# rojas-diego/tokengeex

Measured on NVIDIA B200. Metric: encode_input_throughput, higher is better.
Workload: dtype f64 scores / u32 ids

## Files before the change

### tokengeex_b200/csrc/tgx_api.cu

```cuda
#include <cub/cub.cuh>
#include <cuda_runtime.h>

#include <algorithm>
#include <cmath>
#include <cstdio>
#include <cstdlib>
#include <cstring>
#include <ctime>
#include <memory>
#include <mutex>
#include <string>
#include <thread>
#include <vector>

#include "../../include/tokengeex_b200.h"
#include "tgx_kernels.cuh"
#include "tgx_match_kernels.cuh"
#include "tgx_team_kernel.cuh"
#include "tgx_fb_rows_kernels.cuh"
#include "trie_build.h"

namespace {

thread_local std::string g_err;
// ... 704 lines not shown
  if (m->device < 0) return TGX_OK;
  cudaStream_t st = m->w().stream;
  tgx::TokenHash h;
  bool hash_ok = V != 0 && max_token_len >= 1 && max_token_len <= 16;
  if (hash_ok && built) {
    hash_ok = built_err->empty();
    if (hash_ok) h = std::move(*built);
  } else if (hash_ok) {
    hash_ok = tgx::build_token_hash(token_bytes, token_offsets, V, &h).empty();
  }
  if (hash_ok) CU(m->d_hash.reserve(h.slots.size() * sizeof(tgx::Slot)));
  m->hash.mask = 0;
  m->hash.slots.clear();
  m->have_rows = false;
  if (hash_ok) {
    CU(cudaMemcpyAsync(m->d_hash.p, h.slots.data(), h.slots.size() * sizeof(tgx::Slot), cudaMemcpyHostToDevice, st));
    CU(cudaStreamSynchronize(st));
    m->hash = std::move(h);
  }
  return TGX_OK;
}

int ensure_match_tables(tgx_model* m) {
  if (m->have_rows || m->device < 0) return TGX_OK;
  if (!tgx::build_match_tables(&m->da).empty()) return TGX_OK;
  const tgx::DoubleArray& da = m->da;
  cudaStream_t st = m->w().stream;
  CU(m->d_trie8.reserve(da.slots8.size() * 8));
  CU(m->d_rows.reserve(da.rows.size() * 8 + 256));
  CU(m->d_rowids.reserve(da.row_ids.size() * 4 + 256));
  CU(cudaMemcpyAsync(m->d_trie8.p, da.slots8.data(), da.slots8.size() * 8, cudaMemcpyHostToDevice, st));
  CU(cudaMemcpyAsync(m->d_rows.p, da.rows.data(), da.rows.size() * 8, cudaMemcpyHostToDevice, st));
  CU(cudaMemcpyAsync(m->d_rowids.p, da.row_ids.data(), da.row_ids.size() * 4, cudaMemcpyHostToDevice, st));
  CU(m->d_pair2.reserve(da.pair2.size() * 8));
  CU(cudaMemcpyAsync(m->d_pair2.p, da.pair2.data(), da.pair2.size() * 8, cudaMemcpyHostToDevice, st));
  CU(cudaStreamSynchronize(st));
  m->have_rows = true;
  m->rows16 = (uint32_t)(da.rows.size() / 2);
  return TGX_OK;
}

int run_crlf(tgx_model* m, const uint8_t* d_text, const uint64_t* d_off, uint64_t S, uint64_t N) {
  cudaStream_t st = m->w().stream;
  uint64_t n_tiles = (N + CRLF_TILE - 1) / CRLF_TILE;
  CU(m->w().text2.reserve(N + 16));
  CU(m->w().off2.reserve((S + 1) * 8));
  CU(m->w().bitmap.reserve((N / 32 + 4) * 4));
  CU(m->w().blk.reserve((n_tiles + 1) * 8 * 2));
  CU(dev_fill(m->w().bitmap.p, 0, (N / 32 + 4) * 4, st));
  if (S > 1) {
    crlf_mark_starts<<<nblk(S, 256), 256, 0, st>>>(d_off, S, m->w().bitmap.as<uint32_t>());
    m->w().stats.launches += 1;
  }
  unsigned long long* removed = m->w().blk.as<unsigned long long>();
  unsigned long long* prefix = removed + n_tiles + 1;
  CU(dev_fill(removed, 0, (n_tiles + 1) * 8, st));
  if (n_tiles) {
    crlf_count<<<(uint32_t)n_tiles, CRLF_BLOCK, 0, st>>>(d_text, N, m->w().bitmap.as<uint32_t>(), removed);
    m->w().stats.launches += 1;
  }
  size_t tmp = 0;
  CU(cub::DeviceScan::ExclusiveSum(nullptr, tmp, removed, prefix, (int)(n_tiles + 1), st));
  CU(m->w().cubtmp.reserve(tmp));
  CU(cub::DeviceScan::ExclusiveSum(m->w().cubtmp.p, tmp, removed, prefix, (int)(n_tiles + 1), st));
  m->w().stats.launches += 2;
  if (n_tiles) {
    crlf_scatter<<<(uint32_t)n_tiles, CRLF_BLOCK, 0, st>>>(d_text, N, d_off, S, m->w().bitmap.as<uint32_t>(), prefix,
                                                          n_tiles, m->w().text2.as<uint8_t>(), m->w().off2.as<uint64_t>());
    m->w().stats.launches += 1;
  } else {
    CU(dev_fill(m->w().off2.p, 0, (S + 1) * 8, st));
  }
  CU(cudaGetLastError());
  return TGX_OK;
}

int sort_units(tgx_model* m, uint32_t U) {
  CU(m->w().keys_out.reserve((size_t)U * 4 + 4));
  CU(m->w().vals_out.reserve((size_t)U * 4 + 4));
  size_t tmp = 0;
  CU(cub::DeviceRadixSort::SortPairsDescending(nullptr, tmp, m->w().ulen.as<uint32_t>(), m->w().keys_out.as<uint32_t>(),
                                               m->w().vals_in.as<uint32_t>(), m->w().vals_out.as<uint32_t>(), (int)U, 0, 32,
                                               m->w().stream));
  CU(m->w().cubtmp.reserve(tmp));
  CU(cub::DeviceRadixSort::SortPairsDescending(m->w().cubtmp.p, tmp, m->w().ulen.as<uint32_t>(), m->w().keys_out.as<uint32_t>(),
                                               m->w().vals_in.as<uint32_t>(), m->w().vals_out.as<uint32_t>(), (int)U, 0, 32,
                                               m->w().stream));
  m->w().stats.launches += 4;
  return TGX_OK;
}

int read_words(tgx_model* m, const void* d0, const void* d1, unsigned long long* o0, unsigned long long* o1);

int run_match(tgx_model* m, const uint8_t* d_text, uint64_t N, const uint8_t* d_skip = nullptr) {
  cudaStream_t st = m->w().stream;
  CU(m->w().rec.reserve((N + 64) * 4));
  MatchParams mp;
  mp.text = d_text;
  mp.blob_end = d_text + N;
  mp.N = N;
  mp.trie8 = m->d_trie8.as<uint2>();
  mp.root_base = m->da.root_base;
  mp.rec = m->w().rec.as<uint32_t>();
  mp.skip = d_skip;
  mp.pair2 = m->d_pair2.as<uint2>();
  mp.slice = 0;
  const size_t budget = (size_t)std::min<int64_t>(m->match_stage_bytes, (int64_t)m->smem_optin - 1024);
  mp.staged = (uint32_t)std::min<size_t>(m->da.slots8.size(), budget / 8);
  const size_t smem = (size_t)mp.staged * 8;
  auto launch = [&](auto kernel, int ilp) -> cudaError_t {
    const uint32_t threads = (uint32_t)std::min(m->match_threads, mk_max_threads(ilp));
    cudaError_t e = cudaFuncSetAttribute(kernel, cudaFuncAttributeMaxDynamicSharedMemorySize, (int)smem);
    if (e != cudaSuccess) return e;
    const uint64_t per_cta = (uint64_t)threads * ilp;
    const uint64_t want = (uint64_t)m->num_sms * (uint64_t)std::max(1, m->match_ctas_per_sm);
    const uint64_t rounds = std::max<uint64_t>(1, (N + per_cta * want - 1) / (per_cta * want));
    mp.slice = rounds * per_cta;
    const uint32_t grid = (uint32_t)((N + mp.slice - 1) / mp.slice);
    kernel<<<grid, threads, smem, st>>>(mp);
    return cudaGetLastError();
  };
  if (m->match_compact) {
    const uint32_t threads = MK2_THREADS;
    const size_t qbytes = (size_t)(threads / 32) * 2 * MK2_Q * 8;
    const size_t budget2 = (size_t)std::min<int64_t>(m->match_stage_bytes, (int64_t)m->smem_optin - 1024 - (int64_t)qbytes);
    mp.staged = (uint32_t)std::min<size_t>(m->da.slots8.size(), budget2 / 8);
    const size_t smem2 = (size_t)mp.staged * 8 + qbytes;
    CU(cudaFuncSetAttribute(match2_kernel, cudaFuncAttributeMaxDynamicSharedMemorySize, (int)smem2));
    const uint64_t per_cta = (uint64_t)threads * 4;
    const uint64_t want = (uint64_t)m->num_sms * (uint64_t)std::max(1, m->match_ctas_per_sm);
    const uint64_t rounds = std::max<uint64_t>(1, (N + per_cta * want - 1) / (per_cta * want));
    mp.slice = rounds * per_cta;
    match2_kernel<<<(uint32_t)((N + mp.slice - 1) / mp.slice), threads, smem2, st>>>(mp);
    CU(cudaGetLastError());
    m->w().stats.launches += 1;
    return TGX_OK;
  }
  CU(launch(match_kernel<4>, 4));
  m->w().stats.launches += 1;
  return TGX_OK;
}

int run_viterbi(tgx_model* m, const uint8_t* d_text, const uint64_t* d_off, uint64_t S, uint64_t N,
                uint64_t* d_proc_len, bool with_dropout = false) {
  cudaStream_t st = m->w().stream;
  if (S >= (1ull << 32)) return fail(TGX_ERR_INVALID, "too many samples in one call (< 2^32)");
  uint32_t U = (uint32_t)S;
  const uint64_t n_tiles = (N + EM_TILE - 1) / EM_TILE;
  CU(m->w().ustart.reserve((size_t)U * 8 + 8));
  CU(m->w().ulen.reserve((size_t)U * 4 + 4));
  CU(m->w().vals_in.reserve((size_t)U * 4 + 4));
  CU(m->w().bp.reserve(N + 64));
  CU(m->w().mark.reserve(n_tiles * EM_TILE + 64));
  CU(m->w().ntok.reserve(((size_t)U + 1) * 8));
  CU(m->w().status.reserve((size_t)U * 4 + 4));
  CU(m->w().small.reserve(256));
  units_from_samples<<<nblk(U, 256), 256, 0, st>>>(d_off, S, m->w().ustart.as<uint64_t>(), m->w().ulen.as<uint32_t>(),
                                                  m->w().vals_in.as<uint32_t>(), d_proc_len);
  m->w().stats.launches += 1;
  int rc = sort_units(m, U);
  if (rc) return rc;
  uint32_t* counts = m->w().small.as<uint32_t>();
  uint32_t thr = (uint32_t)std::min<int64_t>(m->long_threshold, 0x7FFFFFFF);
  const uint32_t thr2 = (uint32_t)std::min<int64_t>(m->team_long_threshold, 0x7FFFFFFF);
  split_sorted<<<1, 32, 0, st>>>(m->w().keys_out.as<uint32_t>(), U, thr, thr2, counts);
  m->w().stats.launches += 1;
  CU(dev_fill(m->w().ntok.p, 0, ((size_t)U + 1) * 8, st));
  CU(dev_fill(m->w().status.p, 0, (size_t)U * 4 + 4, st));
  CU(dev_fill(m->w().mark.p, 0, n_tiles * EM_TILE, st));

  UnitParams u;
  u.text = d_text;
  u.unit_start = m->w().ustart.as<uint64_t>();
  u.unit_len = m->w().ulen.as<uint32_t>();
  u.order = m->w().vals_out.as<uint32_t>();
  u.trie = m->d_trie;
  u.root_base = m->da.root_base;
  u.rows = std::max<uint32_t>(1, m->da.max_token_len);
  u.W = u.rows + 1;
  u.counts = counts;
  u.first = 0;
  u.count = U;

  const double dropout = with_dropout ? m->dropout : 0.0;
  const int algo_req = m->algo == 4 ? (with_dropout && N >= m->wide_bytes && u.rows <= 16 ? 3 : 2) : m->algo;
  if (!(dropout > 0.0) && (algo_req == 0 || algo_req == 3) && u.rows <= 16) {
    rc = ensure_match_tables(m);
    if (rc) return rc;
  }
  const int algo = dropout > 0.0 ? (algo_req == 1 ? 1 : 2) : ((algo_req == 0 || algo_req == 3) && !m->have_rows ? 2 : algo_req);
  m->w().algo_used = algo;
  m->w().side_used = false;
  uint32_t n_long = 0;
  if (algo == 3 && u.rows <= 16 && N && U) {
    unsigned long long w01 = 0, w23 = 0;
    rc = read_words(m, counts, counts + 2, &w01, &w23);
    if (rc) return rc;
    n_long = std::min<uint32_t>((uint32_t)w23, (uint32_t)(w01 >> 32));
  }
  CU(cudaEventRecord(m->w().ev[8], st));
  if ((algo == 0 || algo == 3) && u.rows <= 16 && N) {
    const uint8_t* d_skip = nullptr;
    if (algo == 3 && n_long && m->match_compact && m->match_skip) {
      const size_t nb = (size_t)((N + 127) >> 7);
      CU(m->w().skip.reserve(nb + 64));
      CU(dev_fill(m->w().skip.p, 0, nb, st));
      mark_skip_kernel<<<nblk((uint64_t)n_long * 32, 256), 256, 0, st>>>(u.unit_start, u.unit_len, u.order, n_long,
                                                                        m->w().skip.as<uint8_t>());
      m->w().stats.launches += 1;
      d_skip = m->w().skip.as<uint8_t>();
    }
    rc = run_match(m, d_text, N, d_skip);
    if (rc) return rc;
  }
  CU(cudaEventRecord(m->w().ev[9], st));
  CU(cudaEventRecord(m->w().ev[0], st));
  if (algo == 3 && u.rows <= 16) {
    if (N && U) {
      const uint32_t per_cta = (uint32_t)std::max(1, m->side_load);
      const uint32_t P = n_long ? std::min<uint32_t>((n_long + per_cta - 1) / per_cta, (uint32_t)m->num_sms * 2u / 3u) : 0u;
      unsigned int* ctr = m->w().small.as<unsigned int>() + 8;
      CU(dev_fill(ctr, 0, 8, st));
      CU(cudaEventRecord(m->w().ev_side_fork, st));
      if (P) {
        CU(cudaStreamWaitEvent(m->w().stream_side, m->w().ev_side_fork, 0));
        PairParams pp;
        pp.u = u;
        pp.u.part = 3;
        pp.u.count = n_long;
        pp.blob_end = d_text + N;
        pp.bp = m->w().bp.as<uint8_t>();
        pp.counter = ctr;
        pp.dbg = 0;
        m->w().side_used = true;
        CU(cudaEventRecord(m->w().ev[10], m->w().stream_side));
        {
          cudaStream_t keep = m->w().stream;
          m->w().stream = m->w().stream_side;
          m->pair_grid_cap = P;
          const int keep_groups = m->groups;
          if (m->side_groups > 0) m->groups = m->groups > 0 ? std::min(m->groups, m->side_groups) : m->side_groups;
          cudaError_t e = launch_viterbi_pair_r<2>(m, pp, 0);
          m->groups = keep_groups;
          m->pair_grid_cap = 0;
          m->w().stream = keep;
          CU(e);
        }
        CU(cudaEventRecord(m->w().ev[11], m->w().stream_side));
        CU(cudaEventRecord(m->w().ev_side_join, m->w().stream_side));
        CU(cudaStreamWaitEvent(m->w().stream_low, m->w().ev_side_fork, 0));
      }
      TeamParams tm;
      tm.u = u;
      tm.u.part = 4;
      tm.u.count = U - std::min(U, n_long);
      tm.rec = m->w().rec.as<uint32_t>();
      tm.rows = m->d_rows.as<double>();
      tm.bp = m->w().bp.as<uint8_t>();
      tm.counter = m->w().small.as<unsigned int>() + 9;
      const size_t budget = (size_t)std::min<int64_t>(m->team_hot_bytes, (int64_t)m->smem_optin - 1024);
      tm.hot16 = (uint32_t)std::max<size_t>(std::min<size_t>(m->rows16, budget / 16), std::min<size_t>(m->rows16, 9));
      const size_t smem = (size_t)tm.hot16 * 16;
      const uint32_t n_short = tm.u.count;
      if (n_short) {
        constexpr uint32_t warps = TM_WARPS, per_warp = 8;
        CU(cudaFuncSetAttribute(viterbi_team_kernel<warps>, cudaFuncAttributeMaxDynamicSharedMemorySize, (int)smem));
        const uint32_t ctas = ((n_short + per_warp - 1) / per_warp + warps - 1) / warps;
        const uint32_t g1 = std::max<uint32_t>(1, std::min<uint32_t>(ctas, (uint32_t)m->num_sms - P));
        viterbi_team_kernel<warps><<<g1, warps * 32, smem, st>>>(tm);
        m->w().stats.launches += 1;
        if (P && ctas > g1) {
          viterbi_team_kernel<warps><<<std::min<uint32_t>(ctas - g1, P), warps * 32, smem, m->w().stream_low>>>(tm);
          m->w().stats.launches += 1;
        }
        CU(cudaGetLastError());
      }
      if (P) {
        CU(cudaEventRecord(m->w().ev_low_join, m->w().stream_low));
        CU(cudaStreamWaitEvent(st, m->w().ev_low_join, 0));
      }
    }
  } else if (algo == 0 && u.rows <= 16) {
    if (N && U) {
      RowsParams rp;
      rp.u = u;
      rp.u.part = 0;
      rp.rec = m->w().rec.as<uint32_t>();
      rp.rows = m->d_rows.as<double>();
      const size_t budget = (size_t)std::min<int64_t>(m->rows_hot_bytes, (int64_t)m->smem_optin - 1024);
      rp.hot16 = (uint32_t)std::min<size_t>(m->rows16, budget / 16);
      rp.bp = m->w().bp.as<uint8_t>();
      rp.counter = m->w().small.as<unsigned int>() + 8;
      const size_t smem = (size_t)rp.hot16 * 16;
      CU(cudaFuncSetAttribute(viterbi_rows_kernel, cudaFuncAttributeMaxDynamicSharedMemorySize, (int)smem));
      CU(dev_fill(rp.counter, 0, 4, st));
      const uint32_t warps = (uint32_t)std::max(1, std::min(16, m->rows_warps));
      const uint32_t grid = (uint32_t)std::min<uint64_t>(((uint64_t)U + 2 * warps - 1) / (2 * warps), (uint64_t)m->num_sms);
      viterbi_rows_kernel<<<grid, warps * 32, smem, st>>>(rp);
      m->w().stats.launches += 1;
      CU(cudaGetLastError());
    }
  } else if (algo == 2 && u.rows <= 16) {
    PairParams p;
    p.u = u;
    p.u.part = 0;
    p.blob_end = d_text + N;
    p.bp = m->w().bp.as<uint8_t>();
    p.counter = m->w().small.as<unsigned int>() + 8;
    p.dbg = 0;
    DropInfo di;
    di.dropout = dropout;
    di.seed = m->drop_seed;
    di.unit_base = m->drop_unit_base;
    if (!p.u.count) {
    } else {
      CU(launch_viterbi_pair_r<2>(m, p, N, di));
    }
  } else {
    ViterbiParams p;
    p.u = u;
    p.bp = m->w().bp.as<uint8_t>();
    p.dropout = dropout;
    p.drop_seed = m->drop_seed;
    p.unit_base = m->drop_unit_base;
    p.u.part = 1;
    CU(launch_viterbi_g(m, 32, p));
    p.u.part = 2;
    CU(launch_viterbi_g(m, m->g_short, p));
  }
  CU(cudaEventRecord(m->w().ev[1], st));
  if (m->w().side_used) CU(cudaStreamWaitEvent(st, m->w().ev_side_join, 0));
  CU(cudaEventRecord(m->w().ev[12], st));
  CU(cudaEventRecord(m->w().ev[2], st));
  if (U) {
    BacktrackParams b;
    b.unit_start = u.unit_start;
    b.unit_len = u.unit_len;
    b.order = u.order;
    b.counts = counts;
    b.first = 0;
    b.count = U;
    b.bp = m->w().bp.as<uint8_t>();
    b.mark = m->w().mark.as<uint8_t>();
    b.n_tokens = m->w().ntok.as<unsigned long long>();
    b.status = m->w().status.as<int32_t>();
    b.part = 1;
    backtrack_warp_kernel<<<nblk(U, BW_WARPS), BW_WARPS * 32, 0, st>>>(b);
    b.part = 2;
    backtrack_thread_kernel<<<nblk(U, BT_THREADS), BT_THREADS, 0, st>>>(b);
    m->w().stats.launches += 2;
    CU(cudaGetLastError());
  }
  CU(cudaEventRecord(m->w().ev[3], st));
  return TGX_OK;
}

int run_emit(tgx_model* m, const uint8_t* d_text, uint64_t N, uint32_t* d_ids, uint64_t ids_cap,
             unsigned long long* d_freq) {
  cudaStream_t st = m->w().stream;
  const uint64_t n_tiles = (N + EM_TILE - 1) / EM_TILE;
  CU(cudaEventRecord(m->w().ev[4], st));
  if (n_tiles) {
    CU(m->w().tilecnt.reserve((n_tiles + 1) * 16));
    unsigned long long* cnt = m->w().tilecnt.as<unsigned long long>();
    unsigned long long* prefix = cnt + n_tiles + 1;
    const uint32_t grid = (uint32_t)std::min<uint64_t>(n_tiles, (uint64_t)m->num_sms * 8);
    mark_count_kernel<<<grid, EM_BLOCK, 0, st>>>(m->w().mark.as<uint4>(), n_tiles, cnt);
    size_t tmp = 0;
    CU(cub::DeviceScan::ExclusiveSum(nullptr, tmp, cnt, prefix, (int)n_tiles, st));
    CU(m->w().cubtmp.reserve(tmp));
    CU(cub::DeviceScan::ExclusiveSum(m->w().cubtmp.p, tmp, cnt, prefix, (int)n_tiles, st));
    EmitParams e;
    e.mark = m->w().mark.as<uint4>();
    e.text = d_text;
    e.text_bytes = N;
    e.n_tiles = n_tiles;
    e.tile_prefix = prefix;
    e.trie = m->d_trie;
    e.root_base = m->da.root_base;
    e.ids = d_ids;
    e.cap = ids_cap;
    e.freq = d_freq;
    e.V = (uint32_t)m->V;
    const bool use_hash = m->emit_hash && m->hash.mask != 0;
    e.hash = use_hash ? m->d_hash.as<uint4>() : nullptr;
    e.hash_mask = use_hash ? m->hash.mask : 0;
    e.hash_seed = m->hash.seed;
    emit_kernel<<<grid, EM_BLOCK, d_freq ? EM_HOT * 4 : 0, st>>>(e);
    m->w().stats.launches += 4;
    CU(cudaGetLastError());
  }
  CU(cudaEventRecord(m->w().ev[5], st));
  return TGX_OK;
}

int read_words(tgx_model* m, const void* d0, const void* d1, unsigned long long* o0, unsigned long long* o1) {
  CU(cudaEventRecord(m->w().ev_ctl, m->w().stream));
  CU(cudaStreamWaitEvent(m->w().stream_ctl, m->w().ev_ctl, 0));
  if (d0) CU(cudaMemcpyAsync(m->w().h_words, d0, 8, cudaMemcpyDeviceToHost, m->w().stream_ctl));
  if (d1) CU(cudaMemcpyAsync(m->w().h_words + 1, d1, 8, cudaMemcpyDeviceToHost, m->w().stream_ctl));
  CU(cudaStreamSynchronize(m->w().stream_ctl));
  if (d0 && o0) *o0 = m->w().h_words[0];
  if (d1 && o1) *o1 = m->w().h_words[1];
  return TGX_OK;
}

int first_bad(tgx_model* m, uint32_t U, int64_t* out_idx, const void* extra = nullptr, unsigned long long* extra_out = nullptr) {
  unsigned long long* d = m->w().small.as<unsigned long long>() + 2;
  CU(dev_fill(d, 0xFF, 8, m->w().stream));
  if (U) {
    first_bad_unit<<<nblk(U, 256), 256, 0, m->w().stream>>>(m->w().status.as<int32_t>(), U, d);
    m->w().stats.launches += 1;
  }
  unsigned long long h = ~0ull;
  int rc = read_words(m, d, extra, &h, extra_out);
  if (rc) return rc;
  *out_idx = (h == ~0ull) ? -1 : (int64_t)h;
  return TGX_OK;
}

void finish_stats(tgx_model* m, int which) {
  float ms = 0;
  if (cudaEventElapsedTime(&ms, m->w().ev[0], m->w().ev[1]) == cudaSuccess) {
    if (which == 1) m->w().stats.viterbi_ms = ms;
    if (which == 2) m->w().stats.fwd_ms = ms;
  }
  if (which == 2 && cudaEventElapsedTime(&ms, m->w().ev[2], m->w().ev[3]) == cudaSuccess) m->w().stats.bwd_ms = ms;
  if (which == 1 && cudaEventElapsedTime(&ms, m->w().ev[2], m->w().ev[3]) == cudaSuccess) m->w().stats.back_ms = ms;
  if (which == 1 && cudaEventElapsedTime(&ms, m->w().ev[4], m->w().ev[5]) == cudaSuccess) m->w().stats.emit_ms = ms;
  if (which == 1 && cudaEventElapsedTime(&ms, m->w().ev[8], m->w().ev[9]) == cudaSuccess) m->w().stats.match_ms = ms;
  if (which == 1 && cudaEventElapsedTime(&ms, m->w().ev[8], m->w().ev[12]) == cudaSuccess) m->w().stats.forward_ms = ms;
  if (which == 1) m->w().stats.algo = m->w().algo_used;
  if (which == 1 && m->w().side_used && cudaEventElapsedTime(&ms, m->w().ev[10], m->w().ev[11]) == cudaSuccess) m->w().stats.side_ms = ms;
  if (cudaEventElapsedTime(&ms, m->w().ev[6], m->w().ev[7]) == cudaSuccess) m->w().stats.total_ms = ms;
  m->last_stats = m->w().stats;
}

}

extern "C" {

const char* tgx_last_error(void) { return g_err.c_str(); }

int tgx_model_create(const uint8_t* token_bytes, const uint64_t* token_offsets, const double* scores,
                     uint64_t vocab_size, int device, tgx_model** out) {
  if (!out || !token_offsets || (!token_bytes && vocab_size && token_offsets[vocab_size]) || (!scores && vocab_size))
    return fail(TGX_ERR_INVALID, "null argument");
  std::unique_ptr<tgx_model> m(new tgx_model());
  std::string err = tgx::build_double_array(token_bytes, token_offsets, scores, vocab_size, &m->da);
  if (!err.empty()) return fail(TGX_ERR_UNSUPPORTED, err);
  m->V = vocab_size;
  m->V_built = vocab_size;
  m->device = device;
  if (device >= 0) {
    int n = 0;
    if (cudaGetDeviceCount(&n) != cudaSuccess || device >= n)
      return fail(TGX_ERR_NO_DEVICE, "CUDA device " + std::to_string(device) + " not available");
    CU(cudaSetDevice(device));
    CU(cudaDeviceGetAttribute(&m->num_sms, cudaDevAttrMultiProcessorCount, device));
    CU(cudaDeviceGetAttribute(&m->smem_optin, cudaDevAttrMaxSharedMemoryPerBlockOptin, device));
    CU(cudaMemcpyToSymbol(tgxk::c_exp_hdr, TGX_EXP_HDR, sizeof(TGX_EXP_HDR)));
    CU(cudaMemcpyToSymbol(tgxk::c_log_hdr, TGX_LOG_HDR, sizeof(TGX_LOG_HDR)));
    CU(cudaMemcpyToSymbol(tgxk::c_exp_tab, TGX_EXP_TAB, sizeof(TGX_EXP_TAB)));
    CU(cudaMemcpyToSymbol(tgxk::c_log_tab, TGX_LOG_TAB, sizeof(TGX_LOG_TAB)));
    for (auto& w : m->ws) {
      CU(cudaStreamCreateWithFlags(&w.stream, cudaStreamNonBlocking));
      CU(cudaStreamCreateWithFlags(&w.stream_ctl, cudaStreamNonBlocking));
      CU(cudaEventCreateWithFlags(&w.ev_ctl, cudaEventDisableTiming));
      {
        int lo = 0, hi = 0;
        CU(cudaDeviceGetStreamPriorityRange(&lo, &hi));
        CU(cudaStreamCreateWithPriority(&w.stream_side, cudaStreamNonBlocking, hi));
        CU(cudaStreamCreateWithPriority(&w.stream_low, cudaStreamNonBlocking, lo));
      }
      CU(cudaEventCreateWithFlags(&w.ev_low_join, cudaEventDisableTiming));
      CU(cudaEventCreateWithFlags(&w.ev_side_fork, cudaEventDisableTiming));
      CU(cudaEventCreateWithFlags(&w.ev_side_join, cudaEventDisableTiming));
      CU(cudaHostAlloc(reinterpret_cast<void**>(&w.h_words), 64, cudaHostAllocDefault));
      for (auto& e : w.ev) CU(cudaEventCreate(&e));
    }
    CU(cudaStreamCreateWithFlags(&m->stream2, cudaStreamNonBlocking));
    CU(cudaStreamCreateWithFlags(&m->stream3, cudaStreamNonBlocking));
    CU(cudaStreamCreateWithFlags(&m->stream4, cudaStreamNonBlocking));
    CU(cudaStreamCreateWithFlags(&m->stream5, cudaStreamNonBlocking));
    CU(cudaStreamCreateWithFlags(&m->stream6, cudaStreamNonBlocking));
    CU(cudaEventCreateWithFlags(&m->ev_join6, cudaEventDisableTiming));
    for (auto& e : m->ev_grp) CU(cudaEventCreateWithFlags(&e, cudaEventDisableTiming));
    CU(cudaEventCreateWithFlags(&m->ev_join5, cudaEventDisableTiming));
    CU(cudaEventCreateWithFlags(&m->ev_join3, cudaEventDisableTiming));
    CU(cudaEventCreateWithFlags(&m->ev_join4, cudaEventDisableTiming));
    CU(cudaStreamCreateWithFlags(&m->stream_h2d, cudaStreamNonBlocking));
    CU(cudaStreamCreateWithFlags(&m->stream_d2h, cudaStreamNonBlocking));
    for (int i = 0; i < 2; i++) {
      CU(cudaEventCreateWithFlags(&m->ev_h2d[i], cudaEventDisableTiming));
      CU(cudaEventCreateWithFlags(&m->ev_d2h[i], cudaEventDisableTiming));
      for (auto& e : m->ev_split[i]) CU(cudaEventCreate(&e));
    }
    CU(cudaEventCreateWithFlags(&m->ev_fork, cudaEventDisableTiming));
    CU(cudaEventCreateWithFlags(&m->ev_join, cudaEventDisableTiming));
    CU(cudaEventCreateWithFlags(&m->ev_caller, cudaEventDisableTiming));
    size_t bytes = m->da.slots.size() * sizeof(tgx::Slot);
    CU(cudaMalloc(&m->d_trie, bytes));
    m->trie_cap = m->da.slots.size();
    CU(cudaMemcpyAsync(m->d_trie, m->da.slots.data(), bytes, cudaMemcpyHostToDevice, m->w().stream));
    CU(cudaStreamSynchronize(m->w().stream));
    int rc = upload_aux_tables(m.get(), m->da, token_bytes, token_offsets, vocab_size, m->da.max_token_len);
    if (rc) return rc;
  }
  *out = m.release();
  return TGX_OK;
}

int tgx_model_rebuild(tgx_model* m, const uint8_t* token_bytes, const uint64_t* token_offsets, const double* scores,
                      uint64_t vocab_size) {
  if (!m || !token_offsets || (!token_bytes && vocab_size && token_offsets[vocab_size]) || (!scores && vocab_size))
    return fail(TGX_ERR_INVALID, "null argument");
  std::lock_guard<std::recursive_mutex> g(m->mu);
  tgx::TokenHash hash;
  std::string hash_err = "not built";
  std::thread hash_thread;
  if (m->device >= 0 && vocab_size)
    hash_thread = std::thread([&] { hash_err = tgx::build_token_hash(token_bytes, token_offsets, vocab_size, &hash); });
  struct Joiner {
    std::thread& t;
    ~Joiner() {
      if (t.joinable()) t.join();
    }
  } joiner{hash_thread};
  tgx::DoubleArray fresh;
  std::string err = "miss";
  if (m->retarget_permille > 0 && m->V_built && vocab_size * 1000ull >= m->V_built * (uint64_t)m->retarget_permille)
    err = tgx::retarget_double_array(&m->da, token_bytes, token_offsets, scores, vocab_size);
  const bool in_place = err.empty();
  if (err == "miss") {
    err = tgx::build_double_array(token_bytes, token_offsets, scores, vocab_size, &fresh, false);
    if (err.empty()) m->V_built = vocab_size;
  }
  if (!err.empty()) return fail(TGX_ERR_UNSUPPORTED, err);
  if (!in_place) m->da = std::move(fresh);
  m->V = vocab_size;
  const tgx::DoubleArray& da = m->da;
  if (m->device >= 0) {
// ... 1315 lines not shown
```

### tokengeex_b200/csrc/tgx_kernels.cuh

```cuda
#pragma once
#include <cstdint>
#include <cuda_runtime.h>

#include "tgx_libm.h"
#include "tgx_libm_tables.h"
#include "trie_build.h"

namespace tgxk {

constexpr uint32_t NONE = 0xFFFFFFFFu;
constexpr uint32_t F_TERM = 2u << 24, F_HASCH = 4u << 24, ID_MASK = 0x00FFFFFFu;
constexpr int ROW_STRIDE = 33;
constexpr int WPB = 4;

struct UnitParams {
  const uint8_t* text;
  const uint64_t* unit_start;
  const uint32_t* unit_len;
  const uint32_t* order;
  uint32_t first, count;
  const uint32_t* counts;
  int part;
  const uint4* trie;
  uint32_t root_base;
// ... 285 lines not shown
  }
}

__device__ __forceinline__ void pair_consume(const double* __restrict__ tb, int g, double& best, uint32_t& ps,
                                             uint32_t& len0, uint32_t& len1) {
  double sc[4];
  sc[0] = tb[0];
  sc[1] = tb[PT_ROW];
  uint32_t sv_hi = 0, sv_ps = 0;
#pragma unroll
  for (int j = 0; j < 32; j++) {
    if (j + 2 < 32) sc[(j + 2) & 3] = tb[(j + 2) * PT_ROW];
    const double bs = __shfl_sync(0xFFFFFFFFu, best, j & 15, 16);
    const bool own = g == (j & 15);
    if (own) {
      sv_hi = (uint32_t)__double2hiint(best);
      sv_ps = ps;
    }
    const double cand = __dadd_rn(bs, sc[j & 3]);
    if (cand > best || own) {
      best = cand;
      ps = j;
    }
    if ((j & 15) == 15) {
      const uint32_t l = (sv_hi == 0xFFF00000u) ? 0u : (((uint32_t)(j - 15 + g) - sv_ps) & 31u);
      if (j == 15) len0 = l; else len1 = l;
    }
  }
}

template <int R, int HOT, bool DROP = false>
__device__ __forceinline__ void pair_body(const PairParams& p, unsigned char* smem, const DropInfo* di = nullptr) {
  constexpr int WG = 2 * R + 1;
  const UnitParams& u = p.u;
  const int lane = threadIdx.x & 31, warp = threadIdx.x >> 5;
  const int grp = warp / WG, wg = warp % WG;
  const bool spare = (uint32_t)grp >= p.groups;
  const int h = lane >> 4, g = lane & 15;
  const double ninf = __longlong_as_double(0xFFF0000000000000ll);

  const uint4* hot = reinterpret_cast<const uint4*>(smem);
  unsigned char* gbase = smem + (size_t)p.hot_slots * 16 + (size_t)grp * pair_group_bytes(R);
  double* tab = reinterpret_cast<double*>(gbase);
  PairInfo* s_info = reinterpret_cast<PairInfo*>(gbase + (size_t)2 * 2 * R * PT_TILE * 8);
  if (HOT > 0) {
    uint4* hw = reinterpret_cast<uint4*>(smem);
    for (uint32_t i = threadIdx.x; i < p.hot_slots; i += blockDim.x) hw[i] = __ldg(u.trie + i);
  }

  double best = ninf;
  uint32_t ps = 0;
  unsigned long long pw[3] = {0, 0, 0};
  uint32_t psh = 0, pf_tile = 0;
  int32_t pf_unit = -1;
  PairInfo cur;
  cur.unit = -1; cur.start = 0; cur.n = 0; cur.tile0 = 0; cur.ntiles = 0; cur.pad[0] = cur.pad[1] = 0;
  uint32_t ufirst = u.first, ucount = u.count;
  unit_range(u.counts, u.part, ufirst, ucount);
  auto fetch = [&]() {
    const uint32_t idx = atomicAdd(p.counter, 1u);
    if (idx < ucount) {
      cur.unit = (int32_t)u.order[ufirst + idx];
      cur.n = u.unit_len[cur.unit];
      cur.start = u.unit_start[cur.unit];
      cur.tile0 = 0;
      cur.ntiles = cur.n / 32 + 1;
    } else {
      cur.unit = -1;
    }
  };
  if (!spare && wg == 0 && g == 0) {
    fetch();
    s_info[0 * 2 + h] = cur;
    PairInfo none = cur;
    none.unit = -1;
    s_info[3 * 2 + h] = none;
  }
  __syncthreads();
  if (spare) return;

  for (uint32_t r = 0;; r++) {
    if (wg == 0) {
      if (g == 0) {
        if (cur.unit >= 0) {
          cur.tile0 += R;
          if (cur.tile0 >= cur.ntiles) fetch();
        }
        s_info[((r + 1) & 3) * 2 + h] = cur;
      }
      const PairInfo ci = s_info[((r + 3) & 3) * 2 + h];
#pragma unroll
      for (int k = 0; k < R; k++) {
        const uint32_t t = ci.tile0 + k;
        const bool act = ci.unit >= 0 && t < ci.ntiles;
        if (act && t == 0) {
          best = (g == 0) ? 0.0 : ninf;
          ps = 0;
        }
        const double* tb = tab + ((size_t)(((r + 1) & 1) * 2 + h) * R + k) * PT_TILE + g;
        uint32_t len0, len1;
        if (p.dbg & 2u) { len0 = len1 = 1; } else
        pair_consume(tb, g, best, ps, len0, len1);
        if (act) {
          const uint32_t e0 = t * 32 + g, e1 = e0 + 16;
          if (e0 >= 1 && e0 <= ci.n) p.bp[ci.start + e0 - 1] = (uint8_t)len0;
          if (e1 <= ci.n) p.bp[ci.start + e1 - 1] = (uint8_t)len1;
        }
      }
    } else {
      const int w = wg - 1;
      const int ph = w & 1, k = w >> 1;
      const PairInfo pi = s_info[(r & 3) * 2 + ph];
      const uint32_t t = pi.tile0 + k;
      if (pi.unit >= 0 && t < pi.ntiles) {
        const uint32_t pos = t * 32 + lane;
        double* row = tab + ((size_t)((r & 1) * 2 + ph) * R + k) * PT_TILE + lane * PT_ROW;
        const uint8_t* ptr = u.text + pi.start + pos;
        if (!(pf_unit == pi.unit && pf_tile == t)) load_window(ptr, p.blob_end, pw, psh);
        unsigned long long w3[3] = {pw[0], pw[1], pw[2]};
        const uint32_t sh = psh;
        if (t + R < pi.ntiles) {
          load_window(ptr + 32 * R, p.blob_end, pw, psh);
          pf_unit = pi.unit;
          pf_tile = t + R;
        } else {
          pf_unit = -1;
        }
        if constexpr (DROP)
          pair_produce<HOT, true>(u.trie, hot, u.root_base, w3, sh, pos < pi.n, row, lane, di->dropout,
                                  drop_unit_key(di->seed, di->unit_base + (uint32_t)pi.unit), pos);
        else
          pair_produce<HOT>(u.trie, hot, u.root_base, w3, sh, pos < pi.n && !(p.dbg & 1u), row, lane);
      }
    }
    asm volatile("bar.sync %0, %1;" ::"r"(grp + 1), "r"(WG * 32) : "memory");
    const bool more = s_info[(r & 3) * 2 + 0].unit >= 0 || s_info[(r & 3) * 2 + 1].unit >= 0 ||
                      s_info[((r + 1) & 3) * 2 + 0].unit >= 0 || s_info[((r + 1) & 3) * 2 + 1].unit >= 0;
    if (!more) break;
  }
}

template <int R, int HOT, int MAXT>
__global__ void __launch_bounds__(MAXT, 1) viterbi_pair_kernel(PairParams p) {
  extern __shared__ __align__(16) unsigned char smem[];
  pair_body<R, HOT>(p, smem);
}

template <int R, int HOT, int MAXT>
__global__ void __launch_bounds__(MAXT, 1) viterbi_pair_drop_kernel(PairParams p, DropInfo di) {
  extern __shared__ __align__(16) unsigned char smem[];
  pair_body<R, HOT, true>(p, smem, &di);
}

struct BacktrackParams {
  const uint64_t* unit_start;
  const uint32_t* unit_len;
  const uint32_t* order;
  uint32_t first, count;
  const uint32_t* counts;
  int part;
  const uint8_t* bp;
  uint8_t* mark;
  unsigned long long* n_tokens;
  int32_t* status;
};

constexpr int BT_THREADS = 128;

__global__ void __launch_bounds__(BT_THREADS) backtrack_thread_kernel(BacktrackParams p) {
  const uint32_t i = blockIdx.x * blockDim.x + threadIdx.x;
  uint32_t pfirst = p.first, pcount = p.count;
  unit_range(p.counts, p.part, pfirst, pcount);
  if (i >= pcount) return;
  const uint32_t unit = p.order[pfirst + i];
  const uint32_t n = p.unit_len[unit];
  const uint64_t start = p.unit_start[unit];
  const uint8_t* b = p.bp + start;
  uint8_t* mk = p.mark + start;
  unsigned long long k = 0;
  int st = 0;
  if (n > 0) {
    if (__ldg(b + n - 1) == 0) {
      st = 6;
    } else {
      uint32_t pos = n;
      while (pos > 0) {
        const uint32_t l = __ldg(b + pos - 1);
        if (l == 0 || l > pos) { st = 99; break; }
        mk[pos - 1] = (uint8_t)l;
        pos -= l;
        k++;
      }
    }
  }
  p.n_tokens[unit] = st ? 0ull : k;
  p.status[unit] = st;
}

constexpr int BW_WARPS = 8;
constexpr int BW_CHUNK = 1024;
constexpr int BW_VECS = 72;
constexpr int BW_SEG_STRIDE = 34;

__global__ void __launch_bounds__(BW_WARPS * 32) backtrack_warp_kernel(BacktrackParams p) {
  __shared__ __align__(16) uint8_t s_len[BW_WARPS][BW_VECS * 16];
  __shared__ int16_t s_exit[BW_WARPS][32 * BW_SEG_STRIDE];
  const int lane = threadIdx.x & 31, w = threadIdx.x >> 5;
  const uint32_t i = blockIdx.x * BW_WARPS + w;
  uint32_t pfirst = p.first, pcount = p.count;
  unit_range(p.counts, p.part, pfirst, pcount);
  if (i >= pcount) return;
  const uint32_t unit = p.order[pfirst + i];
  const uint32_t n = p.unit_len[unit];
  const uint64_t start = p.unit_start[unit];
  const uint4* b16 = reinterpret_cast<const uint4*>(p.bp);
  uint8_t* sl = s_len[w];
  int16_t* ex = s_exit[w] + lane * BW_SEG_STRIDE;
  unsigned long long k = 0;
  int st = 0;
  if (n == 0) {
    if (lane == 0) { p.n_tokens[unit] = 0; p.status[unit] = 0; }
    return;
  }
  uint64_t gtop = start + n - 1;
  uint64_t gbase = (gtop - start >= BW_CHUNK) ? gtop - (BW_CHUNK - 1) : start;
  uint64_t wbase = gbase & ~15ull;
  uint4 v[3];
#pragma unroll
  for (int j = 0; j < 3; j++) {
    const uint32_t vi = lane + 32 * j;
    v[j] = (vi < BW_VECS && wbase + 16ull * vi <= gtop) ? __ldg(b16 + (wbase >> 4) + vi) : make_uint4(0, 0, 0, 0);
  }
  for (;;) {
#pragma unroll
    for (int j = 0; j < 3; j++) {
      const uint32_t vi = lane + 32 * j;
      if (vi < BW_VECS) reinterpret_cast<uint4*>(sl)[vi] = v[j];
    }
    __syncwarp();
    const uint32_t C = (uint32_t)(gtop - gbase) + 1;
    const uint32_t off = (uint32_t)(gbase - wbase);
    if (gtop == start + n - 1 && sl[off + C - 1] == 0) { st = 6; break; }
    const bool last = gbase == start;
    const uint64_t nwbase = (gbase >= 1087 ? gbase - 1087 : 0) & ~15ull;
    if (!last) {
#pragma unroll
      for (int j = 0; j < 3; j++) {
        const uint32_t vi = lane + 32 * j;
        v[j] = (vi < BW_VECS && nwbase + 16ull * vi < gbase) ? __ldg(b16 + (nwbase >> 4) + vi) : make_uint4(0, 0, 0, 0);
      }
    }
    const int lo = 32 * lane;
#pragma unroll 4
    for (int q = 1; q <= 32; q++) {
      const int x = lo + q;
      if (x > (int)C) break;
      const int l = sl[off + x - 1];
      const int t = x - l;
      int e;
      if (l == 0) e = x;
      else if (t <= lo) e = t;
      else e = ex[t - lo];
      ex[q] = (int16_t)e;
    }
    __syncwarp();
    int cur = (int)C, myent = 0;
    while (cur >= 1) {
      const int s = (cur - 1) >> 5;
      if (s == lane) myent = cur;
      const int nxt = (int)s_exit[w][s * BW_SEG_STRIDE + (cur - 32 * s)];
      if (nxt >= cur) { cur = -32768; break; }
      cur = nxt;
    }
    if (cur != -32768) {
      int x = myent;
      while (x > lo) {
        const int l = sl[off + x - 1];
        if (l == 0) break;
        p.mark[gbase + x - 1] = (uint8_t)l;
        k++;
        x -= l;
      }
    }
    __syncwarp();
    const long long pe = (long long)(gbase - start) + cur;
    if (cur == -32768 || cur > 0 || pe < 0) { st = 99; break; }
    if (pe == 0) break;
    gtop = gbase + cur - 1;
    gbase = (gtop - start >= BW_CHUNK) ? gtop - (BW_CHUNK - 1) : start;
    wbase = nwbase;
  }
#pragma unroll
  for (int o = 16; o; o >>= 1) k += __shfl_xor_sync(0xFFFFFFFFu, k, o);
  if (lane == 0) {
    p.n_tokens[unit] = st ? 0ull : k;
    p.status[unit] = st;
  }
}

constexpr int EM_BLOCK = 256;
constexpr int EM_PER_THREAD = 16;
constexpr int EM_TILE = EM_BLOCK * EM_PER_THREAD;
constexpr uint32_t EM_HOT = 4096;

__device__ __forceinline__ uint32_t nonzero_bytes(uint32_t w) {
  return (((w & 0x7F7F7F7Fu) + 0x7F7F7F7Fu) | w) & 0x80808080u;
}

__device__ __forceinline__ uint32_t em_block_scan(uint32_t v, uint32_t* warp_sums, uint32_t& total) {
  const int lane = threadIdx.x & 31, warp = threadIdx.x >> 5;
  uint32_t x = v;
#pragma unroll
  for (int o = 1; o < 32; o <<= 1) {
    uint32_t y = __shfl_up_sync(0xFFFFFFFFu, x, o);
    if (lane >= o) x += y;
  }
  if (lane == 31) warp_sums[warp] = x;
  __syncthreads();
  uint32_t before = 0, tot = 0;
#pragma unroll
  for (int i = 0; i < EM_BLOCK / 32; i++) {
    const uint32_t ws = warp_sums[i];
    if (i < warp) before += ws;
    tot += ws;
  }
  total = tot;
  return before + x - v;
}

__global__ void __launch_bounds__(EM_BLOCK) mark_count_kernel(const uint4* __restrict__ mark, uint64_t n_tiles,
                                                              unsigned long long* __restrict__ tile_cnt) {
  __shared__ uint32_t ws[EM_BLOCK / 32];
  for (uint64_t tile = blockIdx.x; tile < n_tiles; tile += gridDim.x) {
    const uint4 v = mark[tile * EM_BLOCK + threadIdx.x];
    uint32_t c = __popc(nonzero_bytes(v.x)) + __popc(nonzero_bytes(v.y)) + __popc(nonzero_bytes(v.z)) +
                 __popc(nonzero_bytes(v.w));
#pragma unroll
    for (int o = 16; o; o >>= 1) c += __shfl_xor_sync(0xFFFFFFFFu, c, o);
    if ((threadIdx.x & 31) == 0) ws[threadIdx.x >> 5] = c;
    __syncthreads();
    if (threadIdx.x == 0) {
      uint32_t t = 0;
#pragma unroll
      for (int i = 0; i < EM_BLOCK / 32; i++) t += ws[i];
      tile_cnt[tile] = t;
    }
    __syncthreads();
  }
}

struct EmitParams {
  const uint4* mark;
  const uint8_t* text;
  uint64_t text_bytes;
  uint64_t n_tiles;
  const unsigned long long* tile_prefix;
  const uint4* trie;
  uint32_t root_base;
  uint32_t* ids;
  unsigned long long cap;
  unsigned long long* freq;
  uint32_t V;
  const uint4* hash;
  uint32_t hash_mask;
  unsigned long long hash_seed;
};

__global__ void __launch_bounds__(EM_BLOCK) emit_kernel(EmitParams p) {
  __shared__ uint32_t ws[EM_BLOCK / 32];
  __shared__ uint32_t s_tok[EM_TILE];
  __shared__ __align__(16) uint8_t s_text[EM_TILE + 48];
  extern __shared__ uint32_t s_hot[];
  const bool staged = p.hash_mask && (reinterpret_cast<unsigned long long>(p.text) & 15ull) == 0;
  if (p.freq) {
    for (uint32_t i = threadIdx.x; i < EM_HOT; i += EM_BLOCK) s_hot[i] = 0;
    __syncthreads();
  }
  for (uint64_t tile = blockIdx.x; tile < p.n_tiles; tile += gridDim.x) {
    const uint4 v = p.mark[tile * EM_BLOCK + threadIdx.x];
    if (staged) {
      const uint4* t16 = reinterpret_cast<const uint4*>(p.text) + tile * EM_BLOCK;
      const unsigned long long vb = tile * EM_TILE + 16ull * threadIdx.x;
      uint4 tv = make_uint4(0, 0, 0, 0);
      if (vb + 16 <= p.text_bytes) {
        tv = __ldg(t16 + threadIdx.x);
      } else if (vb < p.text_bytes) {
        uint32_t w[4] = {0, 0, 0, 0};
        for (uint32_t k = 0; vb + k < p.text_bytes; k++) w[k >> 2] |= (uint32_t)__ldg(p.text + vb + k) << (8 * (k & 3));
        tv = make_uint4(w[0], w[1], w[2], w[3]);
      }
      reinterpret_cast<uint4*>(s_text)[threadIdx.x + 1] = tv;
      if (threadIdx.x == 0) reinterpret_cast<uint4*>(s_text)[0] = tile ? __ldg(t16 - 1) : make_uint4(0, 0, 0, 0);
    }
    const uint32_t wv[4] = {v.x, v.y, v.z, v.w};
    uint32_t c = 0;
#pragma unroll
    for (int i = 0; i < 4; i++) c += __popc(nonzero_bytes(wv[i]));
    uint32_t total;
    uint32_t o = em_block_scan(c, ws, total);
#pragma unroll
    for (int i = 0; i < 4; i++) {
#pragma unroll
      for (int b = 0; b < 4; b++) {
        const uint32_t l = (wv[i] >> (8 * b)) & 0xFFu;
        if (l) s_tok[o++] = (l << 16) | (uint32_t)(threadIdx.x * EM_PER_THREAD + i * 4 + b);
      }
    }
    __syncthreads();
    const unsigned long long base = p.tile_prefix[tile];
    const uint8_t* tt = p.text + tile * EM_TILE;
    for (uint32_t k = threadIdx.x; k < total; k += EM_BLOCK) {
      const uint32_t tk = s_tok[k];
      const uint32_t len = tk >> 16;
      uint32_t id;
      if (p.hash_mask) {
        unsigned long long lo = 0, hi = 0;
        if (staged) {
          const uint32_t o = 16u + (tk & 0xFFFFu) + 1u - len;
          const uint32_t* w = reinterpret_cast<const uint32_t*>(s_text) + (o >> 2);
          const uint32_t sh = 8u * (o & 3u);
          const uint32_t w0 = w[0], w1 = w[1], w2 = w[2], w3 = w[3], w4 = w[4];
          lo = (unsigned long long)__funnelshift_r(w0, w1, sh) | ((unsigned long long)__funnelshift_r(w1, w2, sh) << 32);
          hi = (unsigned long long)__funnelshift_r(w2, w3, sh) | ((unsigned long long)__funnelshift_r(w3, w4, sh) << 32);
          if (len < 8) {
            lo &= (1ull << (8 * len)) - 1ull;
            hi = 0;
          } else if (len < 16) {
            hi &= (1ull << (8 * (len - 8))) - 1ull;
          }
        } else {
          const uint8_t* q = tt + (tk & 0xFFFFu) + 1 - len;
          for (uint32_t d = 0; d < len && d < 8; d++) lo |= (unsigned long long)__ldg(q + d) << (8 * d);
          for (uint32_t d = 8; d < len; d++) hi |= (unsigned long long)__ldg(q + d) << (8 * (d - 8));
        }
        const unsigned long long key = tgx::token_key(lo, hi, len, p.hash_seed);
        uint32_t s = tgx::token_key_slot(key, p.hash_mask);
        id = NONE;
        for (int it = 0; it < 256; it++) {
          const uint4 e = __ldg(p.hash + s);
          if ((((unsigned long long)e.y << 32) | e.x) == key) { id = e.z; break; }
          if ((e.x | e.y) == 0) break;
          s = (s + 1) & p.hash_mask;
        }
      } else {
        const uint8_t* q = tt + (tk & 0xFFFFu) + 1 - len;
        uint32_t xb = p.root_base;
        uint4 e = make_uint4(0, 0, 0, 0);
        for (uint32_t d = 0; d < len; d++) {
          e = __ldg(p.trie + (xb ^ (0x100u | __ldg(q + d))));
          xb = e.x >> 9;
        }
        id = e.y & ID_MASK;
      }
      if (p.ids && base + k < p.cap) p.ids[base + k] = id;
      if (p.freq) {
        if (id < EM_HOT) atomicAdd(s_hot + id, 1u);
        else atomicAdd(p.freq + id, 1ull);
      }
    }
    __syncthreads();
  }
  if (p.freq) {
    for (uint32_t i = threadIdx.x; i < EM_HOT && i < p.V; i += EM_BLOCK) {
      const uint32_t c = s_hot[i];
      if (c) atomicAdd(p.freq + i, (unsigned long long)c);
    }
  }
}

__constant__ unsigned long long c_exp_hdr[8];
__constant__ unsigned long long c_log_hdr[18];
__constant__ unsigned long long c_exp_tab[256];
__constant__ unsigned long long c_log_tab[256];

struct LibmTabs {
  const uint64_t* et;
  const double* lt;
};

__device__ __forceinline__ LibmTabs stage_libm_tables(unsigned long long* s_et, double* s_lt) {
  for (int i = threadIdx.x; i < 256; i += blockDim.x) {
    s_et[i] = c_exp_tab[i];
    s_lt[i] = __longlong_as_double((long long)c_log_tab[i]);
  }
  __syncthreads();
  LibmTabs t;
  t.et = reinterpret_cast<const uint64_t*>(s_et);
  t.lt = s_lt;
  return t;
}

__device__ __forceinline__ double tgx_exp(double x, const LibmTabs& t) {
  return tgx_exp_impl(x, reinterpret_cast<const double*>(c_exp_hdr), t.et);
}
__device__ __forceinline__ double tgx_log(double x, const LibmTabs& t) {
  return tgx_log_impl(x, reinterpret_cast<const double*>(c_log_hdr), t.lt);
}

__device__ __forceinline__ double log_sum_exp(double x, double y, const LibmTabs& t) {
  double vmin, vmax;
  if (x > y) { vmin = y; vmax = x; } else { vmin = x; vmax = y; }
// ... 426 lines not shown
```

Measured before the change: 32900.

## Fuse per-tile mark counting into backtrack kernels, staging warp marks in shared memory

Removes the separate mark_count_kernel pass over the mark buffer by having the backtrack kernels accumulate per-tile token counts with atomics as they write marks. The warp backtrack kernel now stages marks in a skewed shared-memory buffer and writes them out as 16-byte streaming stores, popcounting each vector to feed the tile counters. The shared length buffer also gets a skewed layout to reduce bank conflicts. In exchange it adds a tilecnt memset, atomics, extra shared memory and partial-vector byte writes at chunk edges.

```diff
diff --git a/tokengeex_b200/csrc/tgx_api.cu b/tokengeex_b200/csrc/tgx_api.cu
--- a/tokengeex_b200/csrc/tgx_api.cu
+++ b/tokengeex_b200/csrc/tgx_api.cu
@@ -880,6 +880,7 @@
   CU(m->w().vals_in.reserve((size_t)U * 4 + 4));
   CU(m->w().bp.reserve(N + 64));
   CU(m->w().mark.reserve(n_tiles * EM_TILE + 64));
+  CU(m->w().tilecnt.reserve((n_tiles + 1) * 16));
   CU(m->w().ntok.reserve(((size_t)U + 1) * 8));
   CU(m->w().status.reserve((size_t)U * 4 + 4));
   CU(m->w().small.reserve(256));
@@ -896,6 +897,7 @@
   CU(dev_fill(m->w().ntok.p, 0, ((size_t)U + 1) * 8, st));
   CU(dev_fill(m->w().status.p, 0, (size_t)U * 4 + 4, st));
   CU(dev_fill(m->w().mark.p, 0, n_tiles * EM_TILE, st));
+  CU(dev_fill(m->w().tilecnt.p, 0, (n_tiles + 1) * 8, st));
 
   UnitParams u;
   u.text = d_text;
@@ -1070,6 +1072,7 @@
     b.count = U;
     b.bp = m->w().bp.as<uint8_t>();
     b.mark = m->w().mark.as<uint8_t>();
+    b.tile_cnt = m->w().tilecnt.as<unsigned long long>();
     b.n_tokens = m->w().ntok.as<unsigned long long>();
     b.status = m->w().status.as<int32_t>();
     b.part = 1;
@@ -1089,11 +1092,9 @@
   const uint64_t n_tiles = (N + EM_TILE - 1) / EM_TILE;
   CU(cudaEventRecord(m->w().ev[4], st));
   if (n_tiles) {
-    CU(m->w().tilecnt.reserve((n_tiles + 1) * 16));
     unsigned long long* cnt = m->w().tilecnt.as<unsigned long long>();
     unsigned long long* prefix = cnt + n_tiles + 1;
     const uint32_t grid = (uint32_t)std::min<uint64_t>(n_tiles, (uint64_t)m->num_sms * 8);
-    mark_count_kernel<<<grid, EM_BLOCK, 0, st>>>(m->w().mark.as<uint4>(), n_tiles, cnt);
     size_t tmp = 0;
     CU(cub::DeviceScan::ExclusiveSum(nullptr, tmp, cnt, prefix, (int)n_tiles, st));
     CU(m->w().cubtmp.reserve(tmp));
@@ -1115,7 +1116,7 @@
     e.hash_mask = use_hash ? m->hash.mask : 0;
     e.hash_seed = m->hash.seed;
     emit_kernel<<<grid, EM_BLOCK, d_freq ? EM_HOT * 4 : 0, st>>>(e);
-    m->w().stats.launches += 4;
+    m->w().stats.launches += 3;
     CU(cudaGetLastError());
   }
   CU(cudaEventRecord(m->w().ev[5], st));
diff --git a/tokengeex_b200/csrc/tgx_kernels.cuh b/tokengeex_b200/csrc/tgx_kernels.cuh
--- a/tokengeex_b200/csrc/tgx_kernels.cuh
+++ b/tokengeex_b200/csrc/tgx_kernels.cuh
@@ -461,6 +461,14 @@
   pair_body<R, HOT, true>(p, smem, &di);
 }
 
+constexpr int EM_BLOCK = 256;
+constexpr int EM_PER_THREAD = 16;
+constexpr int EM_TILE = EM_BLOCK * EM_PER_THREAD;
+
+__device__ __forceinline__ uint32_t nonzero_bytes(uint32_t w) {
+  return (((w & 0x7F7F7F7Fu) + 0x7F7F7F7Fu) | w) & 0x80808080u;
+}
+
 struct BacktrackParams {
   const uint64_t* unit_start;
   const uint32_t* unit_len;
@@ -470,6 +478,7 @@
   int part;
   const uint8_t* bp;
   uint8_t* mark;
+  unsigned long long* tile_cnt;
   unsigned long long* n_tokens;
   int32_t* status;
 };
@@ -493,13 +502,23 @@
       st = 6;
     } else {
       uint32_t pos = n;
+      uint64_t tile = (start + n - 1) / EM_TILE;
+      uint32_t c = 0;
       while (pos > 0) {
         const uint32_t l = __ldg(b + pos - 1);
         if (l == 0 || l > pos) { st = 99; break; }
         mk[pos - 1] = (uint8_t)l;
+        const uint64_t t = (start + pos - 1) / EM_TILE;
+        if (t != tile) {
+          if (c) atomicAdd(p.tile_cnt + tile, (unsigned long long)c);
+          tile = t;
+          c = 0;
+        }
+        c++;
         pos -= l;
         k++;
       }
+      if (c) atomicAdd(p.tile_cnt + tile, (unsigned long long)c);
     }
   }
   p.n_tokens[unit] = st ? 0ull : k;
@@ -510,10 +529,23 @@
 constexpr int BW_CHUNK = 1024;
 constexpr int BW_VECS = 72;
 constexpr int BW_SEG_STRIDE = 34;
+constexpr int BW_MVECS = BW_CHUNK / 16 + 1;
+__device__ __forceinline__ uint32_t bw_skew(uint32_t i) { return i + ((i >> 5) << 2); }
+constexpr int BW_SKEWED = 16 * BW_VECS + 4 * (BW_VECS / 2);
+constexpr int BW_MSKEWED = 16 * BW_MVECS + 4 * (BW_MVECS / 2 + 1);
+__device__ __forceinline__ void bw_put16(uint8_t* buf, uint32_t vi, uint4 v) {
+  uint32_t* w = reinterpret_cast<uint32_t*>(buf + bw_skew(16 * vi));
+  w[0] = v.x; w[1] = v.y; w[2] = v.z; w[3] = v.w;
+}
+__device__ __forceinline__ uint4 bw_get16(const uint8_t* buf, uint32_t vi) {
+  const uint32_t* w = reinterpret_cast<const uint32_t*>(buf + bw_skew(16 * vi));
+  return make_uint4(w[0], w[1], w[2], w[3]);
+}
 
 __global__ void __launch_bounds__(BW_WARPS * 32) backtrack_warp_kernel(BacktrackParams p) {
-  __shared__ __align__(16) uint8_t s_len[BW_WARPS][BW_VECS * 16];
+  __shared__ __align__(16) uint8_t s_len[BW_WARPS][BW_SKEWED];
   __shared__ int16_t s_exit[BW_WARPS][32 * BW_SEG_STRIDE];
+  __shared__ __align__(16) uint8_t s_mark[BW_WARPS][BW_MSKEWED];
   const int lane = threadIdx.x & 31, w = threadIdx.x >> 5;
   const uint32_t i = blockIdx.x * BW_WARPS + w;
   uint32_t pfirst = p.first, pcount = p.count;
@@ -524,6 +556,7 @@
   const uint64_t start = p.unit_start[unit];
   const uint4* b16 = reinterpret_cast<const uint4*>(p.bp);
   uint8_t* sl = s_len[w];
+  uint8_t* sm = s_mark[w];
   int16_t* ex = s_exit[w] + lane * BW_SEG_STRIDE;
   unsigned long long k = 0;
   int st = 0;
@@ -540,16 +573,17 @@
     const uint32_t vi = lane + 32 * j;
     v[j] = (vi < BW_VECS && wbase + 16ull * vi <= gtop) ? __ldg(b16 + (wbase >> 4) + vi) : make_uint4(0, 0, 0, 0);
   }
+  for (uint32_t vi = lane; vi < BW_MVECS; vi += 32) bw_put16(sm, vi, make_uint4(0, 0, 0, 0));
   for (;;) {
 #pragma unroll
     for (int j = 0; j < 3; j++) {
       const uint32_t vi = lane + 32 * j;
-      if (vi < BW_VECS) reinterpret_cast<uint4*>(sl)[vi] = v[j];
+      if (vi < BW_VECS) bw_put16(sl, vi, v[j]);
     }
     __syncwarp();
     const uint32_t C = (uint32_t)(gtop - gbase) + 1;
     const uint32_t off = (uint32_t)(gbase - wbase);
-    if (gtop == start + n - 1 && sl[off + C - 1] == 0) { st = 6; break; }
+    if (gtop == start + n - 1 && sl[bw_skew(off + C - 1)] == 0) { st = 6; break; }
     const bool last = gbase == start;
     const uint64_t nwbase = (gbase >= 1087 ? gbase - 1087 : 0) & ~15ull;
     if (!last) {
@@ -564,7 +598,7 @@
     for (int q = 1; q <= 32; q++) {
       const int x = lo + q;
       if (x > (int)C) break;
-      const int l = sl[off + x - 1];
+      const int l = sl[bw_skew(off + x - 1)];
       const int t = x - l;
       int e;
       if (l == 0) e = x;
@@ -581,15 +615,46 @@
       if (nxt >= cur) { cur = -32768; break; }
       cur = nxt;
     }
+    const uint64_t mbase = gbase & ~15ull;
+    const uint32_t moff = (uint32_t)(gbase - mbase);
     if (cur != -32768) {
       int x = myent;
       while (x > lo) {
-        const int l = sl[off + x - 1];
+        const int l = sl[bw_skew(off + x - 1)];
         if (l == 0) break;
-        p.mark[gbase + x - 1] = (uint8_t)l;
+        sm[bw_skew(moff + x - 1)] = (uint8_t)l;
         k++;
         x -= l;
       }
+    }
+    __syncwarp();
+    {
+      const uint64_t tile0 = gbase / EM_TILE;
+      const uint32_t split = (uint32_t)min((tile0 + 1) * EM_TILE - mbase, (uint64_t)BW_MVECS * 16);
+      const uint32_t nvec = (moff + C + 15) >> 4;
+      uint8_t* mrow = p.mark + mbase;
+      uint32_t cnt = 0;
+      for (uint32_t vi = lane; vi < nvec; vi += 32) {
+        const uint4 mv = bw_get16(sm, vi);
+        const uint32_t ra = 16u * vi;
+        const uint32_t c = __popc(nonzero_bytes(mv.x)) + __popc(nonzero_bytes(mv.y)) + __popc(nonzero_bytes(mv.z)) +
+                           __popc(nonzero_bytes(mv.w));
+        cnt += ra < split ? c : c << 16;
+        if (ra >= moff && ra + 16 <= moff + C) {
+          __stcs(reinterpret_cast<uint4*>(mrow + ra), mv);
+        } else if (c) {
+#pragma unroll 1
+          for (uint32_t j = ra; j < ra + 16; j++) {
+            const uint8_t l = sm[bw_skew(j)];
+            if (l) mrow[j] = l;
+          }
+        }
+        bw_put16(sm, vi, make_uint4(0, 0, 0, 0));
+      }
+#pragma unroll
+      for (int o = 16; o; o >>= 1) cnt += __shfl_xor_sync(0xFFFFFFFFu, cnt, o);
+      if (lane == 0 && (cnt & 0xFFFFu)) atomicAdd(p.tile_cnt + tile0, (unsigned long long)(cnt & 0xFFFFu));
+      if (lane == 1 && (cnt >> 16)) atomicAdd(p.tile_cnt + tile0 + 1, (unsigned long long)(cnt >> 16));
     }
     __syncwarp();
     const long long pe = (long long)(gbase - start) + cur;
@@ -607,14 +672,7 @@
   }
 }
 
-constexpr int EM_BLOCK = 256;
-constexpr int EM_PER_THREAD = 16;
-constexpr int EM_TILE = EM_BLOCK * EM_PER_THREAD;
 constexpr uint32_t EM_HOT = 4096;
-
-__device__ __forceinline__ uint32_t nonzero_bytes(uint32_t w) {
-  return (((w & 0x7F7F7F7Fu) + 0x7F7F7F7Fu) | w) & 0x80808080u;
-}
 
 __device__ __forceinline__ uint32_t em_block_scan(uint32_t v, uint32_t* warp_sums, uint32_t& total) {
   const int lane = threadIdx.x & 31, warp = threadIdx.x >> 5;
@@ -635,27 +693,6 @@
   }
   total = tot;
   return before + x - v;
-}
-
-__global__ void __launch_bounds__(EM_BLOCK) mark_count_kernel(const uint4* __restrict__ mark, uint64_t n_tiles,
-                                                              unsigned long long* __restrict__ tile_cnt) {
-  __shared__ uint32_t ws[EM_BLOCK / 32];
-  for (uint64_t tile = blockIdx.x; tile < n_tiles; tile += gridDim.x) {
-    const uint4 v = mark[tile * EM_BLOCK + threadIdx.x];
-    uint32_t c = __popc(nonzero_bytes(v.x)) + __popc(nonzero_bytes(v.y)) + __popc(nonzero_bytes(v.z)) +
-                 __popc(nonzero_bytes(v.w));
-#pragma unroll
-    for (int o = 16; o; o >>= 1) c += __shfl_xor_sync(0xFFFFFFFFu, c, o);
-    if ((threadIdx.x & 31) == 0) ws[threadIdx.x >> 5] = c;
-    __syncthreads();
-    if (threadIdx.x == 0) {
-      uint32_t t = 0;
-#pragma unroll
-      for (int i = 0; i < EM_BLOCK / 32; i++) t += ws[i];
-      tile_cnt[tile] = t;
-    }
-    __syncthreads();
-  }
 }
 
 struct EmitParams {
```

Result: faster. 33590 (median of 6 runs) (+2.1%).
